# PJLab-ADG/DetZero

Measured on AMD Instinct MI355X. Metric: LiDAR frames/sec (160k pts, 0.1m voxels), higher is better.
Workload: dtype f32 as f16 pairs (hi+lo, 22-bit significand; 3 f16 MFMA per product, f32 accumulate)

## Files before the change

detzero_amd/csrc/pair16.hip:

```cpp
#include "hgemm.h"

namespace dz {

template <class M>
__global__ void k_pair16_from_f32(const float *__restrict__ src, long rows, int c_src, int c_dst, uint4 *__restrict__ dst) {
    const int groups = c_dst / 8;
    const long total = rows * groups;
    for (long idx = (long)blockIdx.x * blockDim.x + threadIdx.x; idx < total; idx += (long)gridDim.x * blockDim.x) {
        const long r = idx / groups;
        const int g = (int)(idx % groups);
        float v[8];
#pragma unroll
        for (int e = 0; e < 8; ++e) v[e] = (g * 8 + e < c_src) ? src[r * c_src + g * 8 + e] : 0.f;
        const float a[4] = {v[0], v[1], v[2], v[3]}, b[4] = {v[4], v[5], v[6], v[7]};
        uint2 h0, l0, h1, l1;
        split4<M>(a, h0, l0);
        split4<M>(b, h1, l1);
        dst[idx * 2] = make_uint4(h0.x, h0.y, h1.x, h1.y);
        dst[idx * 2 + 1] = make_uint4(l0.x, l0.y, l1.x, l1.y);
    }
}

template <class M>
__global__ void k_pair16_to_f32(const uint4 *__restrict__ src, long rows, int c, float *__restrict__ dst) {
// ... 87 lines not shown
}

__global__ __launch_bounds__(256) void k_bev_row_index(const uint32_t *__restrict__ bitmap, const uint32_t *__restrict__ prefix, LevelGeom lg, int pad,
                                                       int feat_rows, int2 *__restrict__ idx) {
    const int hp = lg.h + 2 * pad, wp = lg.w + 2 * pad;
    const long total = (long)lg.b * hp * wp;
    for (long pix = (long)blockIdx.x * blockDim.x + threadIdx.x; pix < total; pix += (long)gridDim.x * blockDim.x) {
        const int xp = (int)(pix % wp), yp = (int)((pix / wp) % hp), b = (int)(pix / ((long)wp * hp));
        const int x = xp - pad, y = yp - pad;
        int r0 = -1, r1 = -1;
        if ((unsigned)x < (unsigned)lg.w && (unsigned)y < (unsigned)lg.h) {
            r0 = bitmap_find(bitmap, prefix, lg.key(b, 0, y, x));
            r1 = bitmap_find(bitmap, prefix, lg.key(b, 1, y, x));
            if (r0 >= feat_rows) r0 = -1;
            if (r1 >= feat_rows) r1 = -1;
        }
        idx[pix] = make_int2(r0, r1);
    }
}

constexpr int BEV_DCAP = 8;
constexpr int BEV_MAX_W = 1024;
static inline __host__ __device__ int bev_slot_words(int tiles_x) { return 3 + tiles_x + tiles_x + 1; }

__global__ __launch_bounds__(256) void k_bev_cover_plan(const int2 *__restrict__ idx, int hp, int wp, int ho, int wo, int tiles_y, int tiles_x, int nl,
                                                        int *__restrict__ slots) {
    __shared__ unsigned char vd[BEV_MAX_W];
    __shared__ unsigned long long busy[BEV_DCAP - 2][BEV_MAX_W / 64];
    const int tid = threadIdx.x, ty = blockIdx.x % tiles_y, b = blockIdx.x / tiles_y, y0 = ty * 8;
    for (int k = tid; k < (BEV_DCAP - 2) * (BEV_MAX_W / 64); k += 256) (&busy[0][0])[k] = 0ull;
    for (int x = tid; x < wo; x += 256) {
        int v = BEV_DCAP - 1;
        for (int r = -nl; r < 8 + nl; ++r) {
            const int y = y0 + r;
            if ((unsigned)y >= (unsigned)ho) continue;
            const int2 e = idx[((size_t)b * hp + y + 1) * wp + x + 1];
            if (e.x >= 0 || e.y >= 0) v = min(v, r < 0 ? -r : r > 7 ? r - 7 : 0);
        }
        vd[x] = (unsigned char)v;
    }
    __syncthreads();
    const int wo64 = (wo + 63) & ~63;
    for (int l = 1; l <= nl; ++l)
        for (int x = tid; x < wo64; x += 256) {
            bool bz = false;
            if (x < wo)
                for (int k = max(0, x - l); k <= min(wo - 1, x + l); ++k) bz |= vd[k] <= l;
            const unsigned long long m = __ballot(bz);
            if ((tid & 63) == 0) busy[l - 1][x >> 6] = m;
        }
    __syncthreads();
    if (tid >= nl) return;
    const unsigned long long *const bm = busy[tid];
    int *const s = slots + ((size_t)blockIdx.x * nl + tid) * bev_slot_words(tiles_x);
    const int nw = wo64 >> 6;
    int n = 0, ns = 0, pos = 0;
    for (;;) {
        int w = pos >> 6, x = wo;
        unsigned long long m = bm[w] & (~0ull << (pos & 63));
        while (!m && ++w < nw) m = bm[w];
        if (m) x = w * 64 + __ffsll(m) - 1;
        if (x > pos) s[3 + tiles_x + ns++] = pos | (x << 16);
        if (x >= wo) break;
        s[3 + n++] = x;
        pos = x + 32;
        if (pos >= wo) break;
    }
    unsigned int gm = 0u;
    for (int tx = 0; tx < tiles_x; ++tx) gm |= (unsigned int)(bm[tx >> 1] >> (32 * (tx & 1))) ? 1u << tx : 0u;
    s[0] = n;
    s[1] = ns;
    s[2] = (int)gm;
}

__global__ __launch_bounds__(64) void k_bev_cover_compact(const int *__restrict__ slots, int n_bands, int tiles_y, int tiles_x, int nl, int *__restrict__ lists,
                                                          int stride) {
    const int lane = threadIdx.x, l = blockIdx.y, first = blockIdx.x * 64, sw = bev_slot_words(tiles_x);
    auto slot = [&](int i) { return slots + ((size_t)i * nl + l) * sw; };
    int before[3] = {0, 0, 0}, total[3] = {0, 0, 0};
    for (int i = lane; i < n_bands; i += 64) {
        const int *s = slot(i);
        const int c[3] = {s[0], s[1], (int)__popc((unsigned int)s[2])};
        for (int k = 0; k < 3; ++k) { total[k] += c[k]; if (i < first) before[k] += c[k]; }
    }
    for (int k = 0; k < 3; ++k)
        for (int d = 32; d >= 1; d >>= 1) { total[k] += __shfl_xor(total[k], d); before[k] += __shfl_xor(before[k], d); }
    const int me = first + lane;
    const bool live = me < n_bands;
    const int *const s = slot(live ? me : 0);
    const int n = live ? s[0] : 0, ns = live ? s[1] : 0;
    const unsigned int gm = live ? (unsigned int)s[2] : 0u;
    int pre[3] = {n, ns, (int)__popc(gm)};
    for (int k = 0; k < 3; ++k) {
        for (int d = 1; d < 64; d <<= 1) { const int t = __shfl_up(pre[k], d); if (lane >= d) pre[k] += t; }
        pre[k] += before[k];
    }
    int *const grid = lists + (size_t)l * stride, *const cover = grid + 2 + n_bands * tiles_x;
    if (blockIdx.x == 0 && lane == 0) {
        grid[0] = total[2];
        grid[1] = n_bands * tiles_x - total[2];
        cover[0] = total[0];
        cover[1] = total[1];
    }
    if (!live) return;
    const int b = me / tiles_y, ty = me % tiles_y;
    int *o = cover + 2 + pre[0] - n;
    for (int k = 0; k < n; ++k) o[k] = tile_xy_pack(b, ty, s[3 + k]);
    o = cover + 2 + total[0] + 2 * (pre[1] - ns);
    for (int k = 0; k < ns; ++k) {
        const int sp = s[3 + tiles_x + k];
        o[2 * k] = tile_xy_pack(b, ty, sp & 0xFFFF);
        o[2 * k + 1] = sp >> 16;
    }
    int run = pre[2] - (int)__popc(gm);
    for (int tx = 0; tx < tiles_x; ++tx) {
        const int id = me * tiles_x + tx;
        if ((gm >> tx) & 1u) grid[2 + run++] = id;
        else grid[2 + total[2] + id - run] = id;
    }
}

constexpr int FILL_DEPTH = 8;
template <class M>
__global__ __launch_bounds__(256) void k_bev_fill_spans(const int *__restrict__ list, int batch, int tiles_y, int tiles_x, int ho, int wo,
                                                        const float *__restrict__ shift, int relu, int cout, float *__restrict__ out, int out_hp, int out_wp,
                                                        int out_cstride, int out_coff, const float *__restrict__ zero_resp) {
    const int n_run = list[0], n_fill = min(list[1], batch * tiles_y * (tiles_x + 1));
    if (n_fill <= 0) return;
    const int *const ent = list + 2 + n_run;
    const bool xy = ent[0] < 0;
    const int lane = threadIdx.x & 63;
    const int y8 = blockIdx.x & 7;
    const int wave = __builtin_amdgcn_readfirstlane((int)((blockIdx.x >> 3) * 4 + (threadIdx.x >> 6))), nwaves = (gridDim.x >> 3) * 4;
    const int ppp = cout / 4;
    const int nseg = (wo + 63) / 64;
    for (int u = wave; u < n_fill * nseg; u += nwaves) {
        const int i = u / nseg, seg = u - i * nseg;
        int b, ty, xs, xe;
        if (xy) {
            tile_xy_unpack(ent[2 * i], b, ty, xs);
            xe = ent[2 * i + 1];
        } else {
            const int t = ent[i];
            xs = (t % tiles_x) * 32, xe = min(xs + 32, wo), ty = (t / tiles_x) % tiles_y, b = t / (tiles_x * tiles_y);
        }
        const int y = ty * 8 + y8;
        if ((unsigned)b >= (unsigned)batch || y >= ho || xs < 0 || xe > wo) continue;
        xs += seg * 64;
        if (xs >= xe) continue;
        xe = min(xe, xs + 64);
        const int np = (xe - xs) * ppp;
        float *const drow = out + (((size_t)b * out_hp + y + 1) * out_wp + xs + 1) * out_cstride + out_coff;
        const uint4 *const srow = zero_resp ? reinterpret_cast<const uint4 *>(zero_resp + ((size_t)(y + 1) * out_wp + xs + 1) * cout) : nullptr;
        for (int p0 = lane; p0 < np; p0 += 64 * FILL_DEPTH) {
            uint4 v[FILL_DEPTH];
#pragma unroll
            for (int k = 0; k < FILL_DEPTH; ++k) {
                const int p = p0 + 64 * k;
                if (p >= np) continue;
                if (srow) { v[k] = srow[p]; continue; }
                const int g = (p % ppp) >> 1;
                float v0[4], v1[4];
#pragma unroll
                for (int e = 0; e < 4; ++e) {
                    const float a = shift ? shift[g * 8 + e] : 0.f, bb = shift ? shift[g * 8 + 4 + e] : 0.f;
                    v0[e] = relu ? fmaxf(a, 0.f) : a;
                    v1[e] = relu ? fmaxf(bb, 0.f) : bb;
                }
                uint2 h0, l0, h1, l1;
// ... 4 lines not shown
#pragma unroll
            for (int k = 0; k < FILL_DEPTH; ++k) {
                const int p = p0 + 64 * k;
                if (p < np) *reinterpret_cast<uint4 *>(drow + (size_t)(p / ppp) * out_cstride + (p % ppp) * 4) = v[k];
            }
        }
    }
}

}

using namespace dz;

extern "C" {

static inline int bev_bands(int batch, int ho) { return batch * ceil_div(ho, 8); }
size_t dz_bev_tile_cover_offset(int batch, int ho, int wo) { return (size_t)bev_bands(batch, ho) * ceil_div(wo, 32) + 2; }
size_t dz_bev_tile_cover_words(int batch, int ho, int wo) {
    const size_t n = bev_bands(batch, ho), tx = ceil_div(wo, 32);
    return dz_bev_tile_cover_offset(batch, ho, wo) + 2 + n * tx + 2 * n * (tx + 1);
}
size_t dz_bev_tile_cover_ws_words(int batch, int ho, int wo, int nlists) { return (size_t)bev_bands(batch, ho) * nlists * bev_slot_words(ceil_div(wo, 32)); }

int dz_bev_tile_cover(const int *idx, int batch, int hp, int wp, int ho, int wo, int nlists, int *lists, int *ws, void *stream_) {
    hipStream_t stream = (hipStream_t)stream_;
    DZ_CHECK_ARG(idx && lists && ws && batch > 0 && ho > 0 && wo > 0 && hp >= ho + 2 && wp >= wo + 2 && nlists >= 1 && nlists <= BEV_DCAP - 2,
                 "dz_bev_tile_cover: bad argument (1 <= nlists <= %d)", BEV_DCAP - 2);
    const int ty = ceil_div(ho, 8), tx = ceil_div(wo, 32), n = batch * ty;
    DZ_CHECK_ARG(wo <= BEV_MAX_W && wo <= TILE_XY_MAX_X && ty <= TILE_XY_MAX_TY && batch <= TILE_XY_MAX_B,
                 "dz_bev_tile_cover: %d frames of %d x %d pixels exceed the list entry (%d frames, %d rows, %d columns)", batch, ho, wo, TILE_XY_MAX_B,
                 TILE_XY_MAX_TY * 8, BEV_MAX_W);
    hipLaunchKernelGGL(k_bev_cover_plan, dim3(n), dim3(256), 0, stream, reinterpret_cast<const int2 *>(idx), hp, wp, ho, wo, ty, tx, nlists, ws);
    hipLaunchKernelGGL(k_bev_cover_compact, dim3(ceil_div(n, 64), nlists), dim3(64), 0, stream, ws, n, ty, tx, nlists, lists,
                       (int)dz_bev_tile_cover_words(batch, ho, wo));
    DZ_LAUNCH_CHECK();
    return DZ_OK;
}

int dz_bev_fill_spans(const int *list, int batch, int ho, int wo, const float *shift, int relu, int cout, float *out, int out_hp, int out_wp,
                      int out_cstride, int out_coff, const float *zero_resp, int math, void *stream_) {
    hipStream_t stream = (hipStream_t)stream_;
    DZ_CHECK_ARG(list && out && batch > 0 && ho > 0 && wo > 0 && cout > 0 && cout % 8 == 0 && out_cstride % 8 == 0 && out_coff % 8 == 0 &&
                 out_hp >= ho + 2 && out_wp >= wo + 2, "dz_bev_fill_spans: bad argument");
    DZ_CHECK_ARG(math == DZ_MATH_F16X2 || math == DZ_MATH_BF16X2 || math == DZ_MATH_F16, "dz_bev_fill_spans: math %d is not a split mode", math);
    const int ty = ceil_div(ho, 8), tx = ceil_div(wo, 32);
    const dim3 grid((4 * device_cus() + 7) / 8 * 8);
    if (math == DZ_MATH_BF16X2)
        hipLaunchKernelGGL(k_bev_fill_spans<MathBF16>, grid, dim3(256), 0, stream, list, batch, ty, tx, ho, wo, shift, relu, cout, out, out_hp, out_wp,
                           out_cstride, out_coff, zero_resp);
    else
        hipLaunchKernelGGL(k_bev_fill_spans<MathF16>, grid, dim3(256), 0, stream, list, batch, ty, tx, ho, wo, shift, relu, cout, out, out_hp, out_wp,
                           out_cstride, out_coff, zero_resp);
    DZ_LAUNCH_CHECK();
    return DZ_OK;
}

int dz_bev_row_index(const uint32_t *bitmap, const uint32_t *prefix, int batch, int d, int h, int w, int layout, int pad, int feat_rows, int *idx,
                     void *stream_) {
    hipStream_t stream = (hipStream_t)stream_;
    DZ_CHECK_ARG(bitmap && prefix && idx && batch > 0 && h > 0 && w > 0 && pad >= 0 && feat_rows >= 0, "dz_bev_row_index: bad argument");
    if (d != 2) { set_error("dz_bev_row_index: %d z slabs (the sparse-input convolution reads exactly 2)", d); return DZ_ERR_UNSUPPORTED; }
    DZ_CHECK_ARG(layout == DZ_LAYOUT_LINEAR || layout == DZ_LAYOUT_BRICK, "dz_bev_row_index: bad layout %d", layout);
    const LevelGeom lg = make_level(batch, d, h, w, layout);
    const long total = (long)batch * (h + 2 * pad) * (w + 2 * pad);
    hipLaunchKernelGGL(k_bev_row_index, dim3(stream_grid(total, 256)), dim3(256), 0, stream, bitmap, prefix, lg, pad, feat_rows, reinterpret_cast<int2 *>(idx));
    DZ_LAUNCH_CHECK();
    return DZ_OK;
}

int dz_pair16_from_f32(const float *src, long rows, int c_src, int c_dst, int math, float *dst, void *stream_) {
    hipStream_t stream = (hipStream_t)stream_;
    DZ_CHECK_ARG(rows >= 0 && c_src >= 1 && c_dst >= c_src && c_dst % 8 == 0, "dz_pair16_from_f32: bad sizes");
    DZ_CHECK_ARG(math == DZ_MATH_F16X2 || math == DZ_MATH_BF16X2, "dz_pair16_from_f32: math %d is not a split mode", math);
    if (rows == 0) return DZ_OK;
    DZ_CHECK_ARG(src && dst, "dz_pair16_from_f32: null pointer");
    const dim3 grid(stream_grid(rows * (c_dst / 8), 256));
    if (math == DZ_MATH_F16X2)
// ... 70 lines not shown
```

detzero_amd/det_modules.py:

```python
import collections
import contextlib
import os
from functools import partial

import numpy as np
import torch
import torch.nn as nn

from . import ops, range_audit
from .lib import DetZeroHipError
from .range_audit import RangeAudit

PACKED_TABLES = bool(os.environ.get('DZ_TUNE_PACKED_TABLES'))

K3, S1, P1 = (3, 3, 3), (1, 1, 1), (1, 1, 1)


def _inference_only(module):
    if module.training:
        raise DetZeroHipError('%s: only the inference path is implemented on the HIP backend '
                              '(call .eval()); training is out of scope' % type(module).__name__)


def fold_bn(bn, conv_bias=None):
# ... 695 lines not shown
        shift=shift.data_ptr() if shift is not None else None,
        batch=batch, ho=ho, wo=wo, in_hp=in_shape[0], in_wp=in_shape[1], in_cstride=in_cstride, in_coff=in_coff,
        cin=cin, kh=ksize, kw=ksize, stride=stride, in_off=in_off,
        out_hp=out_shape[0], out_wp=out_shape[1], out_cstride=out_cstride, out_coff=out_coff,
        out_sy=out_s, out_sx=out_s, out_dy=out_d[0], out_dx=out_d[1],
        groups=groups, cout_pad=cout_pad,
        g_cout=g_cout if g_cout is not None else [cout_pad], g_ooff=g_ooff if g_ooff is not None else [0],
        relu=1 if relu else 0, phase_groups=1 if phase_groups else 0,
        in_rowidx=in_rowidx.data_ptr() if in_rowidx is not None else None, in_row_channels=int(in_row_channels), in_rows=int(in_rows),
        in_tiles=in_tiles.data_ptr() if in_tiles is not None else None)
    if w_limb3 is not None and not math and ops.conv3x3_limb3_supported(desc):
        desc['w'] = w_limb3().data_ptr()
        ops.conv2d(desc, math=math, out_f32=out_f32, tiles=in_tiles, f32_engine='bf16x3')
        return
    if w_limb3g is not None and not math and ops.conv2d_limb3_supported(desc):
        desc['w'] = w_limb3g().data_ptr()
        ops.conv2d(desc, math=math, out_f32=out_f32, tiles=in_tiles, f32_generic='bf16x3')
        return
    ops.conv2d(desc, math=math, out_f32=out_f32, tiles=in_tiles)


class BaseBEVBackbone(_Cached):

    def __init__(self, model_cfg, input_channels):
        super().__init__()
        self.model_cfg = model_cfg
        layer_nums = list(model_cfg.LAYER_NUMS)
        layer_strides = list(model_cfg.LAYER_STRIDES)
        num_filters = list(model_cfg.NUM_FILTERS)
        upsample_strides = list(model_cfg.UPSAMPLE_STRIDES)
        num_upsample_filters = list(model_cfg.NUM_UPSAMPLE_FILTERS)
        assert len(layer_nums) == len(layer_strides) == len(num_filters) == len(upsample_strides)
        c_in_list = [input_channels, *num_filters[:-1]]
        self.blocks = nn.ModuleList()
        self.deblocks = nn.ModuleList()
        for idx in range(len(layer_nums)):
            cur = [nn.ZeroPad2d(1),
                   nn.Conv2d(c_in_list[idx], num_filters[idx], kernel_size=3, stride=layer_strides[idx], padding=0, bias=False),
                   nn.BatchNorm2d(num_filters[idx], eps=1e-3, momentum=0.01), nn.ReLU()]
            for _ in range(layer_nums[idx]):
                cur.extend([nn.Conv2d(num_filters[idx], num_filters[idx], kernel_size=3, padding=1, bias=False),
                            nn.BatchNorm2d(num_filters[idx], eps=1e-3, momentum=0.01), nn.ReLU()])
            self.blocks.append(nn.Sequential(*cur))
            s = upsample_strides[idx]
            if not (isinstance(s, int) and s >= 1):
                raise DetZeroHipError('BaseBEVBackbone: only integer UPSAMPLE_STRIDES >= 1 are supported')
# ... 61 lines not shown
                    if ci == 0:
                        conv_layer(rows, (xh + 2, xw + 2), *self._p(cv, e_in, e_mid, key='w_zmajor'), True, y, (xh + 2, xw + 2), cin=cv['cin'],
                                   in_cstride=xc, ksize=3, stride=1, in_off=0, out_cstride=cv['cout'], out_d=(1, 1), ho=xh, wo=xw, batch=nb0,
                                   math=self.math, in_rowidx=ridx, in_row_channels=rows_c, in_rows=rows.shape[0])
                    else:
                        conv_layer(x, (xh + 2, xw + 2), *self._p(cv, e_mid, e_mid), True, y, (xh + 2, xw + 2), cin=cv['cin'], in_cstride=xc,
                                   ksize=3, stride=1, in_off=0, out_cstride=cv['cout'], out_d=(1, 1), ho=xh, wo=xw, batch=nb0, math=self.math)
                    outs.append(y[:1].clone())
                    x, xc = y, cv['cout']
            for old_key, old_imgs in cache.put(key, outs):
                for st in users.pop(old_key, ()):
                    for img in old_imgs:
                        img.record_stream(st)
                CACHE_GEN[0] += 1
        if torch.cuda.is_current_stream_capturing():
            cache.pin(key)
        elif torch.device(dev).type == 'cuda':
            users.setdefault(key, set()).add(torch.cuda.current_stream(dev))
        return outs

    def _level_convs(self, li, lvl, x, xh, xw, xc, batch, dev, sparse_in=None, out_last=None):
        convs = lvl['convs']
        bufs = None
        tiles = zero = None
        audit = range_audit.active()
        e_in, e_mid = self._e('encoded'), self._e('spatial_features_2d')
        if sparse_in is not None and li == 0 and SKIP_EMPTY_TILES:
            nl = min(len(convs), 6) if all(cv['stride'] == 1 for cv in convs) else 1
            key = ('zero_resp', xh, xw, int(self.math), str(dev), int(batch), e_in, e_mid)
            if nl > 1 and key not in lvl and torch.cuda.is_current_stream_capturing():
                nl = 1
                if not getattr(self, '_warned_capture_nl1', False):
                    self._warned_capture_nl1 = True
                    import warnings
                    warnings.warn('BaseBEVBackbone: graph capture of a %d-frame pass without an eager pass of the same size before it - empty tiles '
                                  'are skipped at the first layer only (run one eager pass first to skip them in all six)' % batch)
            tiles = ops.bev_tile_cover(ops.bev_tile_list(sparse_in[1], xh, xw, nl), batch, xh, xw)
            zero = self._zero_response(lvl, xh, xw, sparse_in[0].shape[1], dev, batch) if nl > 1 else None
        for ci, cv in enumerate(convs):
            s = cv['stride']
            oh, ow = (xh + 2 - 3) // s + 1, (xw + 2 - 3) // s + 1
            if bufs is None:
                bufs = [bordered_zeros('bev2d.l%d.%d' % (li, k), (batch, oh + 2, ow + 2, cv['cout']), dev) for k in range(2)]
            y = out_last if (out_last is not None and ci == len(convs) - 1) else bufs[ci % 2]
            if sparse_in is not None and li == 0 and ci == 0:
                rows, ridx = sparse_in
                wz, scz, shz = self._p(cv, e_in, e_mid, key='w_zmajor')
                conv_layer(rows, (xh + 2, xw + 2), wz, scz, shz, True, y, (oh + 2, ow + 2),
                           cin=cv['cin'], in_cstride=xc, ksize=3, stride=s, in_off=0, out_cstride=cv['cout'],
                           out_d=(1, 1), ho=oh, wo=ow, batch=batch, math=self.math, in_rowidx=ridx, in_row_channels=rows.shape[1],
                           in_rows=rows.shape[0], in_tiles=tiles[0] if tiles is not None else None)
                if tiles is not None:
                    ops.bev_fill_empty_tiles(tiles[0], batch, oh, ow, shz, True, cv['cout'], y, self.math)
            else:
                tl = tiles[ci] if (tiles is not None and ci < tiles.shape[0]) else None
                wc, scc, shc = self._p(cv, e_in if (li == 0 and ci == 0) else e_mid, e_mid)
                conv_layer(x, (xh + 2, xw + 2), wc, scc, shc, True, y, (oh + 2, ow + 2),
                           cin=cv['cin'], in_cstride=xc, ksize=3, stride=s, in_off=0, out_cstride=cv['cout'],
                           out_d=(1, 1), ho=oh, wo=ow, batch=batch, math=self.math, in_tiles=tl, w_limb3=self._l3(cv),
                           w_limb3g=self._l3g(cv))
                if tl is not None:
                    ops.bev_fill_empty_tiles(tl, batch, oh, ow, shc, True, cv['cout'], y, self.math, zero_resp=zero[ci])
            if audit is not None:
                audit.probe('backbone2d.blocks.%d.%d' % (li, 1 + 3 * ci), y, math=self.math, stage='spatial_features_2d', exp=e_mid)
            x, xh, xw, xc = y, oh, ow, cv['cout']
        return x, xh, xw, xc

    def _level_deblock(self, lvl, x, xh, xw, xc, concat, coff, h, w, batch, li=0):
        self._deblock_launches(lvl, x, xh, xw, xc, concat, coff, h, w, batch)
        de = lvl['de']
        audit = range_audit.active()
        if audit is not None:
            audit.probe('backbone2d.deblocks.%d' % li, concat, math=self.math, stage='spatial_features_2d', exp=self._e('spatial_features_2d'),
                        c_off=coff, c=de['cout'])
        return coff + de['cout']

    def _deblock_launches(self, lvl, x, xh, xw, xc, concat, coff, h, w, batch):
        de = lvl['de']
        s = de['s']
        ctot = self.num_bev_features
        e_mid = self._e('spatial_features_2d')
        if xh * s != h or xw * s != w:
            raise DetZeroHipError('BaseBEVBackbone: deblock output %dx%d does not match %dx%d' % (xh * s, xw * s, h, w))
        if self.math and 1 < s * s <= 8 and FUSED_DEBLOCK_PHASES:
# ... 409 lines not shown
```

detzero_amd/lib.py:

```python
import ctypes
import os

import torch

_HERE = os.path.dirname(os.path.abspath(__file__))
LIB_PATH = os.path.join(_HERE, 'libdetzero_hip.so')


ERR_INVALID, ERR_WORKSPACE, ERR_HIP, ERR_UNSUPPORTED = -1, -2, -3, -4


class DetZeroHipError(RuntimeError):
    pass


c_int, c_float, c_size_t, c_void_p, c_double = ctypes.c_int, ctypes.c_float, ctypes.c_size_t, ctypes.c_void_p, ctypes.c_double
c_longlong = ctypes.c_longlong
_I3 = c_int * 3
_F3 = c_float * 3
_F6 = c_float * 6
_I8 = c_int * 8


class Conv2dDesc(ctypes.Structure):
# ... 97 lines not shown
    'dz_spconv_x_windows': (c_int, [c_void_p, c_int, c_void_p, c_int, c_void_p, c_void_p, c_void_p, c_void_p]),
    'dz_build_neighbors_packed_x': (c_int, [c_void_p, c_void_p, c_int, c_void_p, c_void_p, c_int, c_int, c_int, c_int, c_void_p, c_void_p, c_int,
                                            c_void_p, c_void_p, c_void_p, c_void_p]),
    'dz_spconv_forward_split_x': (c_int, [c_void_p, c_int, c_int, c_void_p, c_void_p, c_void_p, c_int, c_int, c_void_p, c_void_p, c_void_p, c_void_p,
                                          c_void_p, c_int, c_void_p, c_int, c_int, c_void_p]),
    'dz_spconv_x_variant': (ctypes.c_char_p, [c_int, c_int]),
    'dz_spconv_forward_x_f32': (c_int, [c_void_p, c_int, c_int, c_void_p, c_void_p, c_void_p, c_int, c_int, c_void_p, c_void_p, c_void_p, c_void_p,
                                        c_void_p, c_int, c_void_p, c_int, c_void_p]),
    'dz_spconv_x_f32_window_rows': (c_int, [c_int, c_int]),
    'dz_spconv_x_f32_variant': (ctypes.c_char_p, [c_int, c_int]),
    'dz_spconv_forward_x_limb3': (c_int, [c_void_p, c_int, c_int, c_void_p, c_void_p, c_void_p, c_int, c_int, c_void_p, c_void_p, c_void_p, c_void_p,
                                          c_void_p, c_int, c_void_p, c_int, c_void_p]),
    'dz_spconv_x_limb3_window_rows': (c_int, [c_int, c_int]),
    'dz_spconv_x_limb3_variant': (ctypes.c_char_p, [c_int, c_int]),
    'dz_spconv_forward_limb3': (c_int, [c_void_p, c_int, c_int, c_void_p, c_void_p, c_int, c_int, c_void_p, c_void_p, c_void_p, c_void_p,
                                        c_void_p, c_int, c_void_p, c_int, c_void_p]),
    'dz_spconv_limb3_tile_rows': (c_int, [c_int, c_int]),
    'dz_spconv_limb3_variant': (ctypes.c_char_p, [c_int, c_int]),
    'dz_bev_tile_cover_words': (c_size_t, [c_int, c_int, c_int]),
    'dz_bev_tile_cover_offset': (c_size_t, [c_int, c_int, c_int]),
    'dz_bev_tile_cover_ws_words': (c_size_t, [c_int, c_int, c_int, c_int]),
    'dz_bev_tile_cover': (c_int, [c_void_p, c_int, c_int, c_int, c_int, c_int, c_int, c_void_p, c_void_p, c_void_p]),
    'dz_bev_fill_spans': (c_int, [c_void_p, c_int, c_int, c_int, c_void_p, c_int, c_int, c_void_p, c_int, c_int, c_int, c_int, c_void_p, c_int, c_void_p]),
    'dz_bev_row_index': (c_int, [c_void_p, c_void_p, c_int, c_int, c_int, c_int, c_int, c_int, c_int, c_void_p, c_void_p]),
    'dz_sparse_to_bev_split': (c_int, [c_void_p, c_void_p, c_void_p, c_int, c_int, c_int, c_int, c_int, c_int, c_void_p,
                                       c_void_p]),
    'dz_sparse_to_bev_split_dense': (c_int, [c_void_p, c_int, c_void_p, c_void_p, c_int, c_int, c_int, c_int, c_int, c_int, c_int, c_void_p,
                                             c_void_p]),
    'dz_conv2d_forward_split': (c_int, [ctypes.POINTER(Conv2dDesc), c_int, c_int, c_void_p]),
    'dz_conv2d_variant_split': (ctypes.c_char_p, [ctypes.POINTER(Conv2dDesc), c_int]),
    'dz_conv3x3_limb3_forward': (c_int, [ctypes.POINTER(Conv2dDesc), c_void_p]),
    'dz_conv3x3_limb3_supported': (c_int, [ctypes.POINTER(Conv2dDesc)]),
    'dz_conv3x3_limb3_variant': (ctypes.c_char_p, [ctypes.POINTER(Conv2dDesc)]),
    'dz_conv2d_limb3_forward': (c_int, [ctypes.POINTER(Conv2dDesc), c_void_p]),
    'dz_conv2d_limb3_supported': (c_int, [ctypes.POINTER(Conv2dDesc)]),
    'dz_conv2d_limb3_variant': (ctypes.c_char_p, [ctypes.POINTER(Conv2dDesc)]),
    'dz_spconv_variant_split': (ctypes.c_char_p, [c_int, c_int]),
    'dz_spconv_variant_split_arm': (ctypes.c_char_p, [c_int, c_int, c_int, c_int, c_size_t]),
    'dz_spconv_variant_split_packed': (ctypes.c_char_p, [c_int, c_int]),
    'dz_xattn_folded_supported': (c_int, [c_int, c_int, c_int]),
    'dz_xattn_folded_workspace_bytes': (ctypes.c_size_t, [c_int, c_int]),
    'dz_xattn_folded': (c_int, [c_void_p] * 6 + [c_int] * 5 + [ctypes.c_float, c_void_p, ctypes.c_size_t, c_void_p, c_void_p]),
    'dz_roi_bev_features': (c_int, [c_void_p, c_int, c_void_p, ctypes.c_long, ctypes.c_long, c_int, c_int, c_int] + [ctypes.c_float] * 4 + [c_int, c_void_p, c_void_p]),
    'dz_linear_splitk_workspace_bytes': (ctypes.c_size_t, [c_int, c_int, c_int]),
    'dz_linear_forward_splitk': (c_int, [c_void_p, c_int, c_int, c_int, c_void_p, c_int, c_int, c_void_p, c_void_p, c_int, c_void_p, c_int, c_int, c_void_p,
                                         ctypes.c_size_t, c_void_p]),
# ... 149 lines not shown
```

detzero_amd/ops.py:

```python
import ctypes
import os
from typing import Callable, NamedTuple, Optional

import numpy as np
import torch

from . import lib as L


def _dev():
    return torch.device('cuda', torch.cuda.current_device())


def _ws(nbytes):
    return torch.empty((max(int(nbytes), 256),), dtype=torch.uint8, device=_dev())


def grid_size_of(pc_range, voxel_size):
    r = np.asarray(pc_range, dtype=np.float32)
    return np.round((r[3:6] - r[0:3]) / np.array(voxel_size)).astype(np.int64)


def voxelize_hard_nosync(points, pc_range, voxel_size, max_points, max_voxels, xy_range_mask=False):
    lib = L.load()
# ... 427 lines not shown
        launch()
    else:
        m = out_level.num_active()
        pairs = table_pairs(nbr, m)
        flops = 2.0 * pairs * cin * cout
        n_in = in_level.num_active() if in_level is not None else m
        nbytes = 4.0 * (n_in * cin + m * cout + nbr.kvol * cin * cout + (m * cout if residual is not None else 0)) + 8.0 * pairs
        PROFILER.wrap(route.variant(cin, cout).decode(), flops, nbytes, launch)
    return out


def bev_row_index(level, feat_rows, pad=1):
    lib = L.load()
    d, h, w = level.shape
    idx = torch.empty((level.batch, h + 2 * pad, w + 2 * pad, 2), dtype=torch.int32, device=level.coords.device)
    rc = lib.dz_bev_row_index(L.ptr(level.bitmap), L.ptr(level.prefix), level.batch, d, h, w, level.layout, pad, int(feat_rows), L.ptr(idx), L.stream())
    L.check(rc, 'dz_bev_row_index')
    return idx


def bev_tile_list(ridx, ho, wo, nlists=1):
    lib = L.load()
    b, hp, wp, _ = ridx.shape
    n = lib.dz_bev_tile_cover_words(b, int(ho), int(wo))
    lst = torch.empty((int(nlists), n), dtype=torch.int32, device=ridx.device)
    ws = torch.empty((lib.dz_bev_tile_cover_ws_words(b, int(ho), int(wo), int(nlists)),), dtype=torch.int32, device=ridx.device)
    L.check(lib.dz_bev_tile_cover(L.ptr(ridx), b, hp, wp, int(ho), int(wo), int(nlists), L.ptr(lst), L.ptr(ws), L.stream()), 'dz_bev_tile_cover')
    return lst


def bev_tile_cover(lists, batch, ho, wo):
    return lists[:, L.load().dz_bev_tile_cover_offset(int(batch), int(ho), int(wo)):]


def bev_fill_empty_tiles(tiles, batch, ho, wo, shift, relu, cout, out, math, zero_resp=None):
    lib = L.load()
    L.check(lib.dz_bev_fill_spans(L.ptr(tiles), int(batch), int(ho), int(wo), L.ptr(shift), 1 if relu else 0, int(cout), L.ptr(out), out.shape[1],
                                  out.shape[2], out.shape[3], 0, L.ptr(zero_resp), int(math), L.stream()), 'dz_bev_fill_spans')


BEV_DENSE = not os.environ.get('DZ_BEV_SCATTER')


def sparse_to_bev(feats, level, c, pad=1, out=None, math=0):
    lib = L.load()
    d, h, w = level.shape
    if out is None:
        out = torch.empty((level.batch, h + 2 * pad, w + 2 * pad, c * d), dtype=torch.float32, device=feats.device)
    if math and d == 2 and c % 8 == 0 and BEV_DENSE:
        rc = lib.dz_sparse_to_bev_split_dense(L.ptr(feats), feats.shape[0], L.ptr(level.bitmap), L.ptr(level.prefix), level.batch, c, d, h, w, level.layout,
                                              pad, L.ptr(out), L.stream())
        L.check(rc, 'dz_sparse_to_bev_split_dense')
        return out
    out.zero_()
    fn = lib.dz_sparse_to_bev_split if math else lib.dz_sparse_to_bev
    rc = fn(L.ptr(feats), L.ptr(level.coords), L.ptr(level.d_m), level.cap, c, d, h, w, pad, L.ptr(out), L.stream())
    L.check(rc, 'dz_sparse_to_bev')
    return out


MATH_MODES = {'f32': 0, 'f16x2': 1, 'bf16x2': 2, 'f16': 3}
# ... 992 lines not shown
```

include/detzero_hip.h:

```cpp
#ifndef DETZERO_HIP_H
#define DETZERO_HIP_H

#include <stddef.h>
#include <stdint.h>

#ifdef __cplusplus
extern "C" {
#endif

#define DZ_OK 0
#define DZ_ERR_INVALID (-1)
#define DZ_ERR_WORKSPACE (-2)
#define DZ_ERR_HIP (-3)
#define DZ_ERR_UNSUPPORTED (-4)

const char *dz_version(void);
const char *dz_last_error(void);
int dz_device_cu_count(void);


size_t dz_voxelize_hard_workspace_bytes(int n, int gx, int gy, int gz, int max_points);
int dz_voxelize_hard(const float *points, int n, int c, const float *h_range6, const float *h_vsize3,
                     const int *h_grid3, int xy_range_mask, int max_points, int max_voxels, float *voxels,
                     int *coords_zyx, int *num_points, int *d_num_voxels, void *ws, size_t ws_bytes,
// ... 124 lines not shown
int dz_spconv_forward_x_f32(const float *in, int in_rows, int cin, const int *nbr_packed, const int *perm, int *windows, int tile_rows,
                            int cap_out, const int *d_m_out, const float *w, const float *scale, const float *shift,
                            const float *residual, int relu, float *out, int cout, void *stream);
int dz_spconv_x_f32_window_rows(int cin, int cout);
const char *dz_spconv_x_f32_variant(int cin, int cout);
int dz_spconv_forward_x_limb3(const float *in, int in_rows, int cin, const int *nbr_packed, const int *perm, int *windows, int tile_rows,
                              int cap_out, const int *d_m_out, const float *w, const float *scale, const float *shift,
                              const float *residual, int relu, float *out, int cout, void *stream);
int dz_spconv_x_limb3_window_rows(int cin, int cout);
const char *dz_spconv_x_limb3_variant(int cin, int cout);
int dz_spconv_forward_limb3(const float *in, int in_rows, int cin, const int *nbr, const uint32_t *tile_masks, int kvol, int cap_out,
                            const int *d_m_out, const float *w_limb, const float *scale, const float *shift, const float *residual,
                            int relu, float *out, int cout, void *stream);
int dz_spconv_limb3_tile_rows(int cin, int cout);
const char *dz_spconv_limb3_variant(int cin, int cout);
int dz_bev_row_index(const uint32_t *bitmap, const uint32_t *prefix, int batch, int d, int h, int w, int layout, int pad, int feat_rows,
                     int *idx, void *stream);
size_t dz_bev_tile_cover_words(int batch, int ho, int wo);
size_t dz_bev_tile_cover_offset(int batch, int ho, int wo);
size_t dz_bev_tile_cover_ws_words(int batch, int ho, int wo, int nlists);
int dz_bev_tile_cover(const int *idx, int batch, int hp, int wp, int ho, int wo, int nlists, int *lists, int *ws, void *stream);
int dz_bev_fill_spans(const int *list, int batch, int ho, int wo, const float *shift, int relu, int cout, float *out, int out_hp, int out_wp,
                      int out_cstride, int out_coff, const float *zero_resp, int math, void *stream);
int dz_sparse_to_bev_split(const float *feats, const int *coords, const int *d_m, int cap, int c, int d, int h,
                           int w, int pad, float *bev, void *stream);
int dz_sparse_to_bev_split_dense(const float *feats, int feat_rows, const uint32_t *bitmap, const uint32_t *prefix, int batch, int c,
                                 int d, int h, int w, int layout, int pad, float *bev, void *stream);
int dz_conv2d_forward_split(const dz_conv2d_desc *h_desc, int math, int out_f32, void *stream);
const char *dz_conv2d_variant_split(const dz_conv2d_desc *h_desc, int out_f32);
int dz_conv3x3_limb3_forward(const dz_conv2d_desc *h_desc, void *stream);
int dz_conv3x3_limb3_supported(const dz_conv2d_desc *h_desc);
const char *dz_conv3x3_limb3_variant(const dz_conv2d_desc *h_desc);
int dz_conv2d_limb3_forward(const dz_conv2d_desc *h_desc, void *stream);
int dz_conv2d_limb3_supported(const dz_conv2d_desc *h_desc);
const char *dz_conv2d_limb3_variant(const dz_conv2d_desc *h_desc);
int dz_linear_forward_split(const float *x, long rows, int cin, int x_stride, const float *w, int cout, int cout_pad, const float *scale,
                            const float *shift, const float *group_shift, int group_rows, int relu, float *y, int y_stride, int math,
                            int out_f32, int group_max, void *stream);
const char *dz_spconv_variant_split(int cin, int cout);
const char *dz_spconv_variant_split_arm(int cin, int cout, int kvol, int has_tile_masks, size_t nbr_bytes);
const char *dz_spconv_variant_split_packed(int cin, int cout);
int dz_xattn_folded_supported(int lq, int e, int heads);
size_t dz_xattn_folded_workspace_bytes(int b, int lk);
int dz_xattn_folded(const float *q, const float *mem, const uint8_t *key_padding_mask, const float *wk_oi, const float *wv_io, const float *bv,
                    int b, int lq, int lk, int e, int heads, float scale, float *workspace, size_t workspace_bytes, float *out, void *stream);
int dz_mlp_chain_forward(const float *x, long rows, const float *wa, const float *sa, const float *ba, const float *group_shift, int ldg, int group_rows,
// ... 217 lines not shown
```

Measured before the change: 1154.

## Fill only empty-tile pixels that the next layer's tiles actually read

```diff
diff --git a/detzero_amd/csrc/pair16.hip b/detzero_amd/csrc/pair16.hip
--- a/detzero_amd/csrc/pair16.hip
+++ b/detzero_amd/csrc/pair16.hip
@@ -133,9 +133,12 @@
 constexpr int BEV_DCAP = 8;
 constexpr int BEV_MAX_W = 1024;
 static inline __host__ __device__ int bev_slot_words(int tiles_x) { return 3 + tiles_x + tiles_x + 1; }
+constexpr int BEV_NEED_PER_GAP = 5;
+static inline __host__ __device__ int bev_need_cap(int tiles_x) { return BEV_NEED_PER_GAP * (tiles_x + 1); }
+static inline __host__ __device__ int bev_slot_words_need(int tiles_x) { return bev_slot_words(tiles_x) + 1 + bev_need_cap(tiles_x); }
 
 __global__ __launch_bounds__(256) void k_bev_cover_plan(const int2 *__restrict__ idx, int hp, int wp, int ho, int wo, int tiles_y, int tiles_x, int nl,
-                                                        int *__restrict__ slots) {
+                                                        int sw, int *__restrict__ slots) {
     __shared__ unsigned char vd[BEV_MAX_W];
     __shared__ unsigned long long busy[BEV_DCAP - 2][BEV_MAX_W / 64];
     const int tid = threadIdx.x, ty = blockIdx.x % tiles_y, b = blockIdx.x / tiles_y, y0 = ty * 8;
@@ -163,7 +166,7 @@
     __syncthreads();
     if (tid >= nl) return;
     const unsigned long long *const bm = busy[tid];
-    int *const s = slots + ((size_t)blockIdx.x * nl + tid) * bev_slot_words(tiles_x);
+    int *const s = slots + ((size_t)blockIdx.x * nl + tid) * sw;
     const int nw = wo64 >> 6;
     int n = 0, ns = 0, pos = 0;
     for (;;) {
@@ -184,25 +187,69 @@
     s[2] = (int)gm;
 }
 
-__global__ __launch_bounds__(64) void k_bev_cover_compact(const int *__restrict__ slots, int n_bands, int tiles_y, int tiles_x, int nl, int *__restrict__ lists,
-                                                          int stride) {
-    const int lane = threadIdx.x, l = blockIdx.y, first = blockIdx.x * 64, sw = bev_slot_words(tiles_x);
+__global__ __launch_bounds__(256) void k_bev_need_plan(int *__restrict__ slots, int n_bands, int tiles_y, int tiles_x, int nl, int sw, int wo) {
+    const int t = blockIdx.x * 256 + threadIdx.x;
+    if (t >= n_bands * (nl - 1)) return;
+    const int i = t / (nl - 1), l = t - i * (nl - 1), ty = i % tiles_y;
+    const int *const own = slots + ((size_t)i * nl + l) * sw, *const nxt = own + sw;
+    int *const need = slots + ((size_t)i * nl + l) * sw + bev_slot_words(tiles_x);
+    const int cap = bev_need_cap(tiles_x);
+    int nn = 0;
+    auto hull = [&](const int *s, int g0, int g1, int &lo, int &hi) {
+        lo = g1, hi = g0;
+        const int n = min(s[0], tiles_x);
+        for (int k = 0; k < n; ++k) {
+            const int a = max(s[3 + k] - 1, g0), e = min(s[3 + k] + 33, g1);
+            if (a < e) lo = min(lo, a), hi = max(hi, e);
+        }
+    };
+    auto emit = [&](int lo, int hi, int r1) {
+        if (lo < hi && nn < cap) need[1 + nn++] = lo | (hi << 11) | (r1 << 22);
+    };
+    const int ng = min(own[1], tiles_x + 1);
+    for (int g = 0; g < ng; ++g) {
+        const int sp = own[3 + tiles_x + g], g0 = sp & 0xFFFF, g1 = min(sp >> 16, wo);
+        int a0, a1, lo, hi;
+        hull(nxt, g0, g1, a0, a1);
+        emit(a0, a1, 0);
+        for (int d = -1; d <= 1; d += 2) {
+            if ((unsigned)(ty + d) >= (unsigned)tiles_y) continue;
+            const int *const nb = nxt + (ptrdiff_t)d * nl * sw;
+            const int r1 = d < 0 ? 1 : 8;
+            if (a0 < a1) {
+                hull(nb, g0, a0, lo, hi);
+                emit(lo, hi, r1);
+                hull(nb, a1, g1, lo, hi);
+                emit(lo, hi, r1);
+            } else {
+                hull(nb, g0, g1, lo, hi);
+                emit(lo, hi, r1);
+            }
+        }
+    }
+    need[0] = nn;
+}
+
+__global__ __launch_bounds__(64) void k_bev_cover_compact(const int *__restrict__ slots, int n_bands, int tiles_y, int tiles_x, int nl, int sw,
+                                                          int *__restrict__ lists, int stride, int *__restrict__ need, int need_stride) {
+    const int lane = threadIdx.x, l = blockIdx.y, first = blockIdx.x * 64, nx = bev_slot_words(tiles_x);
+    const bool needed = need && l < nl - 1;
     auto slot = [&](int i) { return slots + ((size_t)i * nl + l) * sw; };
-    int before[3] = {0, 0, 0}, total[3] = {0, 0, 0};
+    int before[4] = {0, 0, 0, 0}, total[4] = {0, 0, 0, 0};
     for (int i = lane; i < n_bands; i += 64) {
         const int *s = slot(i);
-        const int c[3] = {s[0], s[1], (int)__popc((unsigned int)s[2])};
-        for (int k = 0; k < 3; ++k) { total[k] += c[k]; if (i < first) before[k] += c[k]; }
-    }
-    for (int k = 0; k < 3; ++k)
+        const int c[4] = {s[0], s[1], (int)__popc((unsigned int)s[2]), needed ? s[nx] : 0};
+        for (int k = 0; k < 4; ++k) { total[k] += c[k]; if (i < first) before[k] += c[k]; }
+    }
+    for (int k = 0; k < 4; ++k)
         for (int d = 32; d >= 1; d >>= 1) { total[k] += __shfl_xor(total[k], d); before[k] += __shfl_xor(before[k], d); }
     const int me = first + lane;
     const bool live = me < n_bands;
     const int *const s = slot(live ? me : 0);
-    const int n = live ? s[0] : 0, ns = live ? s[1] : 0;
+    const int n = live ? s[0] : 0, ns = live ? s[1] : 0, nn = live && needed ? s[nx] : 0;
     const unsigned int gm = live ? (unsigned int)s[2] : 0u;
-    int pre[3] = {n, ns, (int)__popc(gm)};
-    for (int k = 0; k < 3; ++k) {
+    int pre[4] = {n, ns, (int)__popc(gm), nn};
+    for (int k = 0; k < 4; ++k) {
         for (int d = 1; d < 64; d <<= 1) { const int t = __shfl_up(pre[k], d); if (lane >= d) pre[k] += t; }
         pre[k] += before[k];
     }
@@ -212,6 +259,10 @@
         grid[1] = n_bands * tiles_x - total[2];
         cover[0] = total[0];
         cover[1] = total[1];
+        if (needed) {
+            need[(size_t)l * need_stride] = 0;
+            need[(size_t)l * need_stride + 1] = total[3];
+        }
     }
     if (!live) return;
     const int b = me / tiles_y, ty = me % tiles_y;
@@ -223,6 +274,14 @@
         o[2 * k] = tile_xy_pack(b, ty, sp & 0xFFFF);
         o[2 * k + 1] = sp >> 16;
     }
+    if (needed) {
+        o = need + (size_t)l * need_stride + 2 + 2 * (pre[3] - nn);
+        for (int k = 0; k < nn; ++k) {
+            const int sp = s[nx + 1 + k];
+            o[2 * k] = tile_xy_pack(b, ty, sp & 0x7FF);
+            o[2 * k + 1] = ((sp >> 11) & 0x7FF) | ((sp >> 22) << 16);
+        }
+    }
     int run = pre[2] - (int)__popc(gm);
     for (int tx = 0; tx < tiles_x; ++tx) {
         const int id = me * tiles_x + tx;
@@ -235,8 +294,8 @@
 template <class M>
 __global__ __launch_bounds__(256) void k_bev_fill_spans(const int *__restrict__ list, int batch, int tiles_y, int tiles_x, int ho, int wo,
                                                         const float *__restrict__ shift, int relu, int cout, float *__restrict__ out, int out_hp, int out_wp,
-                                                        int out_cstride, int out_coff, const float *__restrict__ zero_resp) {
-    const int n_run = list[0], n_fill = min(list[1], batch * tiles_y * (tiles_x + 1));
+                                                        int out_cstride, int out_coff, const float *__restrict__ zero_resp, int per_band) {
+    const int n_run = list[0], n_fill = min(list[1], batch * tiles_y * per_band);
     if (n_fill <= 0) return;
     const int *const ent = list + 2 + n_run;
     const bool xy = ent[0] < 0;
@@ -247,15 +306,17 @@
     const int nseg = (wo + 63) / 64;
     for (int u = wave; u < n_fill * nseg; u += nwaves) {
         const int i = u / nseg, seg = u - i * nseg;
-        int b, ty, xs, xe;
+        int b, ty, xs, xe, r1 = 0;
         if (xy) {
             tile_xy_unpack(ent[2 * i], b, ty, xs);
-            xe = ent[2 * i + 1];
+            xe = ent[2 * i + 1] & 0xFFFF;
+            r1 = (ent[2 * i + 1] >> 16) & 0xF;
         } else {
             const int t = ent[i];
             xs = (t % tiles_x) * 32, xe = min(xs + 32, wo), ty = (t / tiles_x) % tiles_y, b = t / (tiles_x * tiles_y);
         }
-        const int y = ty * 8 + y8;
+        if (r1 && (r1 > 8 || (i & 7) != y8)) continue;
+        const int y = ty * 8 + (r1 ? r1 - 1 : y8);
         if ((unsigned)b >= (unsigned)batch || y >= ho || xs < 0 || xe > wo) continue;
         xs += seg * 64;
         if (xs >= xe) continue;
@@ -306,37 +367,69 @@
 }
 size_t dz_bev_tile_cover_ws_words(int batch, int ho, int wo, int nlists) { return (size_t)bev_bands(batch, ho) * nlists * bev_slot_words(ceil_div(wo, 32)); }
 
-int dz_bev_tile_cover(const int *idx, int batch, int hp, int wp, int ho, int wo, int nlists, int *lists, int *ws, void *stream_) {
+size_t dz_bev_need_words(int batch, int ho, int wo) { return 2 + 2 * (size_t)bev_bands(batch, ho) * bev_need_cap(ceil_div(wo, 32)); }
+size_t dz_bev_tile_cover_need_ws_words(int batch, int ho, int wo, int nlists) {
+    return (size_t)bev_bands(batch, ho) * nlists * bev_slot_words_need(ceil_div(wo, 32));
+}
+
+static int bev_tile_cover(const int *idx, int batch, int hp, int wp, int ho, int wo, int nlists, int *lists, size_t stride, bool need, int *ws,
+                          void *stream_, const char *who) {
     hipStream_t stream = (hipStream_t)stream_;
     DZ_CHECK_ARG(idx && lists && ws && batch > 0 && ho > 0 && wo > 0 && hp >= ho + 2 && wp >= wo + 2 && nlists >= 1 && nlists <= BEV_DCAP - 2,
-                 "dz_bev_tile_cover: bad argument (1 <= nlists <= %d)", BEV_DCAP - 2);
+                 "%s: bad argument (1 <= nlists <= %d)", who, BEV_DCAP - 2);
     const int ty = ceil_div(ho, 8), tx = ceil_div(wo, 32), n = batch * ty;
     DZ_CHECK_ARG(wo <= BEV_MAX_W && wo <= TILE_XY_MAX_X && ty <= TILE_XY_MAX_TY && batch <= TILE_XY_MAX_B,
-                 "dz_bev_tile_cover: %d frames of %d x %d pixels exceed the list entry (%d frames, %d rows, %d columns)", batch, ho, wo, TILE_XY_MAX_B,
+                 "%s: %d frames of %d x %d pixels exceed the list entry (%d frames, %d rows, %d columns)", who, batch, ho, wo, TILE_XY_MAX_B,
                  TILE_XY_MAX_TY * 8, BEV_MAX_W);
-    hipLaunchKernelGGL(k_bev_cover_plan, dim3(n), dim3(256), 0, stream, reinterpret_cast<const int2 *>(idx), hp, wp, ho, wo, ty, tx, nlists, ws);
-    hipLaunchKernelGGL(k_bev_cover_compact, dim3(ceil_div(n, 64), nlists), dim3(64), 0, stream, ws, n, ty, tx, nlists, lists,
-                       (int)dz_bev_tile_cover_words(batch, ho, wo));
-    DZ_LAUNCH_CHECK();
-    return DZ_OK;
-}
-
-int dz_bev_fill_spans(const int *list, int batch, int ho, int wo, const float *shift, int relu, int cout, float *out, int out_hp, int out_wp,
-                      int out_cstride, int out_coff, const float *zero_resp, int math, void *stream_) {
+    const int sw = need ? bev_slot_words_need(tx) : bev_slot_words(tx);
+    hipLaunchKernelGGL(k_bev_cover_plan, dim3(n), dim3(256), 0, stream, reinterpret_cast<const int2 *>(idx), hp, wp, ho, wo, ty, tx, nlists, sw, ws);
+    if (need && nlists > 1)
+        hipLaunchKernelGGL(k_bev_need_plan, dim3(ceil_div(n * (nlists - 1), 256)), dim3(256), 0, stream, ws, n, ty, tx, nlists, sw, wo);
+    hipLaunchKernelGGL(k_bev_cover_compact, dim3(ceil_div(n, 64), nlists), dim3(64), 0, stream, ws, n, ty, tx, nlists, sw, lists, (int)stride,
+                       need ? lists + dz_bev_tile_cover_words(batch, ho, wo) : nullptr, (int)stride);
+    DZ_LAUNCH_CHECK();
+    return DZ_OK;
+}
+
+int dz_bev_tile_cover(const int *idx, int batch, int hp, int wp, int ho, int wo, int nlists, int *lists, int *ws, void *stream) {
+    return bev_tile_cover(idx, batch, hp, wp, ho, wo, nlists, lists, dz_bev_tile_cover_words(batch, ho, wo), false, ws, stream, "dz_bev_tile_cover");
+}
+
+int dz_bev_tile_cover_need(const int *idx, int batch, int hp, int wp, int ho, int wo, int nlists, int *lists, size_t stride, int *ws, void *stream) {
+    DZ_CHECK_ARG(batch > 0 && ho > 0 && wo > 0 && stride >= dz_bev_tile_cover_words(batch, ho, wo) + dz_bev_need_words(batch, ho, wo) &&
+                 stride < (1u << 30), "dz_bev_tile_cover_need: rows of %zu words do not hold the lists and the needed spans", stride);
+    return bev_tile_cover(idx, batch, hp, wp, ho, wo, nlists, lists, stride, true, ws, stream, "dz_bev_tile_cover_need");
+}
+
+static int bev_fill(const int *list, int batch, int ho, int wo, const float *shift, int relu, int cout, float *out, int out_hp, int out_wp,
+                    int out_cstride, int out_coff, const float *zero_resp, int math, void *stream_, bool needed, const char *who) {
     hipStream_t stream = (hipStream_t)stream_;
     DZ_CHECK_ARG(list && out && batch > 0 && ho > 0 && wo > 0 && cout > 0 && cout % 8 == 0 && out_cstride % 8 == 0 && out_coff % 8 == 0 &&
-                 out_hp >= ho + 2 && out_wp >= wo + 2, "dz_bev_fill_spans: bad argument");
-    DZ_CHECK_ARG(math == DZ_MATH_F16X2 || math == DZ_MATH_BF16X2 || math == DZ_MATH_F16, "dz_bev_fill_spans: math %d is not a split mode", math);
+                 out_hp >= ho + 2 && out_wp >= wo + 2, "%s: bad argument", who);
+    DZ_CHECK_ARG(math == DZ_MATH_F16X2 || math == DZ_MATH_BF16X2 || math == DZ_MATH_F16, "%s: math %d is not a split mode", who, math);
     const int ty = ceil_div(ho, 8), tx = ceil_div(wo, 32);
+    const int per_band = needed ? bev_need_cap(tx) : tx + 1;
     const dim3 grid((4 * device_cus() + 7) / 8 * 8);
     if (math == DZ_MATH_BF16X2)
         hipLaunchKernelGGL(k_bev_fill_spans<MathBF16>, grid, dim3(256), 0, stream, list, batch, ty, tx, ho, wo, shift, relu, cout, out, out_hp, out_wp,
-                           out_cstride, out_coff, zero_resp);
+                           out_cstride, out_coff, zero_resp, per_band);
     else
         hipLaunchKernelGGL(k_bev_fill_spans<MathF16>, grid, dim3(256), 0, stream, list, batch, ty, tx, ho, wo, shift, relu, cout, out, out_hp, out_wp,
-                           out_cstride, out_coff, zero_resp);
-    DZ_LAUNCH_CHECK();
-    return DZ_OK;
+                           out_cstride, out_coff, zero_resp, per_band);
+    DZ_LAUNCH_CHECK();
+    return DZ_OK;
+}
+
+int dz_bev_fill_spans(const int *list, int batch, int ho, int wo, const float *shift, int relu, int cout, float *out, int out_hp, int out_wp,
+                      int out_cstride, int out_coff, const float *zero_resp, int math, void *stream) {
+    return bev_fill(list, batch, ho, wo, shift, relu, cout, out, out_hp, out_wp, out_cstride, out_coff, zero_resp, math, stream, false,
+                    "dz_bev_fill_spans");
+}
+
+int dz_bev_fill_needed(const int *list, int batch, int ho, int wo, const float *shift, int relu, int cout, float *out, int out_hp, int out_wp,
+                       int out_cstride, int out_coff, const float *zero_resp, int math, void *stream) {
+    return bev_fill(list, batch, ho, wo, shift, relu, cout, out, out_hp, out_wp, out_cstride, out_coff, zero_resp, math, stream, true,
+                    "dz_bev_fill_needed");
 }
 
 int dz_bev_row_index(const uint32_t *bitmap, const uint32_t *prefix, int batch, int d, int h, int w, int layout, int pad, int feat_rows, int *idx,
diff --git a/detzero_amd/det_modules.py b/detzero_amd/det_modules.py
--- a/detzero_amd/det_modules.py
+++ b/detzero_amd/det_modules.py
@@ -741,6 +741,8 @@
 
 class BaseBEVBackbone(_Cached):
 
+    fill_needed_only = True
+
     def __init__(self, model_cfg, input_channels):
         super().__init__()
         self.model_cfg = model_cfg
@@ -848,7 +850,8 @@
     def _level_convs(self, li, lvl, x, xh, xw, xc, batch, dev, sparse_in=None, out_last=None):
         convs = lvl['convs']
         bufs = None
-        tiles = zero = None
+        tiles = need = zero = None
+        nl = 0
         audit = range_audit.active()
         e_in, e_mid = self._e('encoded'), self._e('spatial_features_2d')
         if sparse_in is not None and li == 0 and SKIP_EMPTY_TILES:
@@ -861,7 +864,10 @@
                     import warnings
                     warnings.warn('BaseBEVBackbone: graph capture of a %d-frame pass without an eager pass of the same size before it - empty tiles '
                                   'are skipped at the first layer only (run one eager pass first to skip them in all six)' % batch)
-            tiles = ops.bev_tile_cover(ops.bev_tile_list(sparse_in[1], xh, xw, nl), batch, xh, xw)
+            lists = ops.bev_tile_list(sparse_in[1], xh, xw, nl)
+            tiles, need = ops.bev_tile_cover(lists, batch, xh, xw), ops.bev_tile_need(lists, batch, xh, xw)
+            if audit is not None or not self.fill_needed_only:
+                need = None
             zero = self._zero_response(lvl, xh, xw, sparse_in[0].shape[1], dev, batch) if nl > 1 else None
         for ci, cv in enumerate(convs):
             s = cv['stride']
@@ -876,7 +882,9 @@
                            cin=cv['cin'], in_cstride=xc, ksize=3, stride=s, in_off=0, out_cstride=cv['cout'],
                            out_d=(1, 1), ho=oh, wo=ow, batch=batch, math=self.math, in_rowidx=ridx, in_row_channels=rows.shape[1],
                            in_rows=rows.shape[0], in_tiles=tiles[0] if tiles is not None else None)
-                if tiles is not None:
+                if tiles is not None and need is not None and nl > 1:
+                    ops.bev_fill_empty_tiles(need[0], batch, oh, ow, shz, True, cv['cout'], y, self.math, needed=True)
+                elif tiles is not None:
                     ops.bev_fill_empty_tiles(tiles[0], batch, oh, ow, shz, True, cv['cout'], y, self.math)
             else:
                 tl = tiles[ci] if (tiles is not None and ci < tiles.shape[0]) else None
@@ -885,7 +893,9 @@
                            cin=cv['cin'], in_cstride=xc, ksize=3, stride=s, in_off=0, out_cstride=cv['cout'],
                            out_d=(1, 1), ho=oh, wo=ow, batch=batch, math=self.math, in_tiles=tl, w_limb3=self._l3(cv),
                            w_limb3g=self._l3g(cv))
-                if tl is not None:
+                if tl is not None and need is not None and ci < nl - 1:
+                    ops.bev_fill_empty_tiles(need[ci], batch, oh, ow, shc, True, cv['cout'], y, self.math, zero_resp=zero[ci], needed=True)
+                elif tl is not None:
                     ops.bev_fill_empty_tiles(tl, batch, oh, ow, shc, True, cv['cout'], y, self.math, zero_resp=zero[ci])
             if audit is not None:
                 audit.probe('backbone2d.blocks.%d.%d' % (li, 1 + 3 * ci), y, math=self.math, stage='spatial_features_2d', exp=e_mid)
diff --git a/detzero_amd/lib.py b/detzero_amd/lib.py
--- a/detzero_amd/lib.py
+++ b/detzero_amd/lib.py
@@ -143,6 +143,10 @@
     'dz_bev_tile_cover_ws_words': (c_size_t, [c_int, c_int, c_int, c_int]),
     'dz_bev_tile_cover': (c_int, [c_void_p, c_int, c_int, c_int, c_int, c_int, c_int, c_void_p, c_void_p, c_void_p]),
     'dz_bev_fill_spans': (c_int, [c_void_p, c_int, c_int, c_int, c_void_p, c_int, c_int, c_void_p, c_int, c_int, c_int, c_int, c_void_p, c_int, c_void_p]),
+    'dz_bev_need_words': (c_size_t, [c_int, c_int, c_int]),
+    'dz_bev_tile_cover_need_ws_words': (c_size_t, [c_int, c_int, c_int, c_int]),
+    'dz_bev_tile_cover_need': (c_int, [c_void_p, c_int, c_int, c_int, c_int, c_int, c_int, c_void_p, c_size_t, c_void_p, c_void_p]),
+    'dz_bev_fill_needed': (c_int, [c_void_p, c_int, c_int, c_int, c_void_p, c_int, c_int, c_void_p, c_int, c_int, c_int, c_int, c_void_p, c_int, c_void_p]),
     'dz_bev_row_index': (c_int, [c_void_p, c_void_p, c_int, c_int, c_int, c_int, c_int, c_int, c_int, c_void_p, c_void_p]),
     'dz_sparse_to_bev_split': (c_int, [c_void_p, c_void_p, c_void_p, c_int, c_int, c_int, c_int, c_int, c_int, c_void_p,
                                        c_void_p]),
diff --git a/detzero_amd/ops.py b/detzero_amd/ops.py
--- a/detzero_amd/ops.py
+++ b/detzero_amd/ops.py
@@ -473,10 +473,11 @@
 def bev_tile_list(ridx, ho, wo, nlists=1):
     lib = L.load()
     b, hp, wp, _ = ridx.shape
-    n = lib.dz_bev_tile_cover_words(b, int(ho), int(wo))
+    n = lib.dz_bev_tile_cover_words(b, int(ho), int(wo)) + lib.dz_bev_need_words(b, int(ho), int(wo))
     lst = torch.empty((int(nlists), n), dtype=torch.int32, device=ridx.device)
-    ws = torch.empty((lib.dz_bev_tile_cover_ws_words(b, int(ho), int(wo), int(nlists)),), dtype=torch.int32, device=ridx.device)
-    L.check(lib.dz_bev_tile_cover(L.ptr(ridx), b, hp, wp, int(ho), int(wo), int(nlists), L.ptr(lst), L.ptr(ws), L.stream()), 'dz_bev_tile_cover')
+    ws = torch.empty((lib.dz_bev_tile_cover_need_ws_words(b, int(ho), int(wo), int(nlists)),), dtype=torch.int32, device=ridx.device)
+    L.check(lib.dz_bev_tile_cover_need(L.ptr(ridx), b, hp, wp, int(ho), int(wo), int(nlists), L.ptr(lst), n, L.ptr(ws), L.stream()),
+            'dz_bev_tile_cover_need')
     return lst
 
 
@@ -484,10 +485,15 @@
     return lists[:, L.load().dz_bev_tile_cover_offset(int(batch), int(ho), int(wo)):]
 
 
-def bev_fill_empty_tiles(tiles, batch, ho, wo, shift, relu, cout, out, math, zero_resp=None):
-    lib = L.load()
-    L.check(lib.dz_bev_fill_spans(L.ptr(tiles), int(batch), int(ho), int(wo), L.ptr(shift), 1 if relu else 0, int(cout), L.ptr(out), out.shape[1],
-                                  out.shape[2], out.shape[3], 0, L.ptr(zero_resp), int(math), L.stream()), 'dz_bev_fill_spans')
+def bev_tile_need(lists, batch, ho, wo):
+    return lists[:-1, L.load().dz_bev_tile_cover_words(int(batch), int(ho), int(wo)):]
+
+
+def bev_fill_empty_tiles(tiles, batch, ho, wo, shift, relu, cout, out, math, zero_resp=None, needed=False):
+    lib = L.load()
+    fn, name = (lib.dz_bev_fill_needed, 'dz_bev_fill_needed') if needed else (lib.dz_bev_fill_spans, 'dz_bev_fill_spans')
+    L.check(fn(L.ptr(tiles), int(batch), int(ho), int(wo), L.ptr(shift), 1 if relu else 0, int(cout), L.ptr(out), out.shape[1], out.shape[2],
+               out.shape[3], 0, L.ptr(zero_resp), int(math), L.stream()), name)
 
 
 BEV_DENSE = not os.environ.get('DZ_BEV_SCATTER')
diff --git a/include/detzero_hip.h b/include/detzero_hip.h
--- a/include/detzero_hip.h
+++ b/include/detzero_hip.h
@@ -170,6 +170,11 @@
 int dz_bev_tile_cover(const int *idx, int batch, int hp, int wp, int ho, int wo, int nlists, int *lists, int *ws, void *stream);
 int dz_bev_fill_spans(const int *list, int batch, int ho, int wo, const float *shift, int relu, int cout, float *out, int out_hp, int out_wp,
                       int out_cstride, int out_coff, const float *zero_resp, int math, void *stream);
+size_t dz_bev_need_words(int batch, int ho, int wo);
+size_t dz_bev_tile_cover_need_ws_words(int batch, int ho, int wo, int nlists);
+int dz_bev_tile_cover_need(const int *idx, int batch, int hp, int wp, int ho, int wo, int nlists, int *lists, size_t stride, int *ws, void *stream);
+int dz_bev_fill_needed(const int *list, int batch, int ho, int wo, const float *shift, int relu, int cout, float *out, int out_hp, int out_wp,
+                       int out_cstride, int out_coff, const float *zero_resp, int math, void *stream);
 int dz_sparse_to_bev_split(const float *feats, const int *coords, const int *d_m, int cap, int c, int d, int h,
                            int w, int pad, float *bev, void *stream);
 int dz_sparse_to_bev_split_dense(const float *feats, int feat_rows, const uint32_t *bitmap, const uint32_t *prefix, int batch, int c,
```

New measurement: 1159, median of 3. No clear change (+0.4%).
